# gopro/cineform-sdk

Hardware: AMD Instinct MI355X
Metric: 1080p YUY2 encode+decode fps (higher is better)
Workload: dtype int16

## Files before the change

cineform-sdk_amd/csrc/cfhd_entropy_gpu.hip:

```cpp
#include "cfhd_entropy_gpu.h"
#include "cfhd_entropy_jobs.h"
#include <hip/hip_runtime.h>
#include <string.h>
#include <stdio.h>
#include <stdlib.h>
#include <algorithm>

namespace cfhd {

int device_init();
int device_current();
namespace { int g_fail(hipError_t e, const char *what) { fprintf(stderr, "[cfhd_amd] %s: %s\n", what, hipGetErrorString(e)); return (int)e ? (int)e : -1; } }
#define HIPCHK(expr) do { hipError_t _e = (expr); if (_e != hipSuccess) return g_fail(_e, #expr); } while (0)

struct GpuEntropyEncoder::Host { EntHostJobs jobs; std::vector<EntHoleGeom> geom; dev::EntFrameJob *frames = nullptr;  };

GpuEntropyEncoder::GpuEntropyEncoder() : host_(new Host) {}
GpuEntropyEncoder::~GpuEntropyEncoder() { release(); delete host_; }

void GpuEntropyEncoder::release()
{
	(void)hipSetDevice(device_);
	void *dev[] = { d_sizes_, d_tables_, d_bands_, d_segband_, d_segs_, d_bandstate_, d_frames_, d_tmpl_, d_packed_, d_offsets_, d_tokens_, d_blocks_, d_masks_ };
	for (void *p : dev) if (p) (void)hipFree(p);
	if (h_samples_) (void)hipHostFree(h_samples_);
	if (h_sizes_) (void)hipHostFree(h_sizes_);
	if (h_offsets_) (void)hipHostFree(h_offsets_);
	d_packed_ = nullptr; d_offsets_ = h_offsets_ = nullptr;
	if (h_tmpl_) (void)hipHostFree(h_tmpl_);
	if (host_->frames) { (void)hipHostFree(host_->frames); host_->frames = nullptr; }
	for (void *&e : ev_) if (e) { (void)hipEventDestroy((hipEvent_t)e); e = nullptr; }
	for (void *&e : ev2_) if (e) { (void)hipEventDestroy((hipEvent_t)e); e = nullptr; }
	if (stream2_) { device_stream_destroy(stream2_); stream2_ = nullptr; }
	timed_ = false;
	h_samples_ = nullptr; d_sizes_ = h_sizes_ = nullptr; d_tables_ = d_bands_ = d_segband_ = d_segs_ = d_bandstate_ = d_frames_ = d_tokens_ = nullptr;
	d_tmpl_ = h_tmpl_ = nullptr; n_ = 0;
	d_blocks_ = nullptr; d_masks_ = nullptr; masks_per_frame_ = 0; use_blocks_ = false;
}

int GpuEntropyEncoder::prepare(const FramePlan &plan, int nframes, int16_t *d_coeffs, size_t stride, size_t sample_cap, void *stream)
{
	group_ = false; plan_ = plan;
	return prepare_units(nframes, d_coeffs, stride, sample_cap, stream);
}

int GpuEntropyEncoder::prepare_group(const GopPlan &plan, int ngroups, int16_t *d_coeffs, size_t stride, size_t sample_cap, void *stream)
{
	group_ = true; gplan_ = plan; plan_ = FramePlan(); plan_.interlaced = false;
	return prepare_units(ngroups, d_coeffs, stride, sample_cap, stream);
}

void GpuEntropyEncoder::build_template(const SampleHeaderInfo &hdr, SampleTemplate *t) const
{
	if (group_) build_group_template(gplan_, hdr, t); else build_sample_template(plan_, hdr, t);
}

int GpuEntropyEncoder::prepare_units(int nframes, int16_t *d_coeffs, size_t stride, size_t sample_cap, void *stream)
{
	int rc = device_init();
	if (rc) return rc;
	release();
	device_ = device_current(); (void)hipSetDevice(device_);
	const FramePlan &plan = plan_;
	n_ = nframes; cap_ = (sample_cap + 255) & ~(size_t)255; stream_ = stream; d_coeffs_ = d_coeffs; coeff_stride_ = stride;
	if (cap_ * (size_t)n_ >= ((size_t)1 << 32)) { fprintf(stderr, "[cfhd_amd] batch of %d frames exceeds the 4 GiB sample arena\n", n_); return -5; }
	{
		std::vector<dev::EntTables> h(2);
		ent_build_tables(&h[0], 1); ent_build_tables(&h[1], 2);
		HIPCHK(hipMalloc(&d_tables_, 2 * sizeof(dev::EntTables)));
		HIPCHK(hipMemcpy(d_tables_, h.data(), 2 * sizeof(dev::EntTables), hipMemcpyHostToDevice));
	}
	SampleHeaderInfo hdr0 = { 1, 2, 2, 4, !plan.interlaced, nullptr, 0, nullptr, 0 };
	tmpl_.assign(n_, SampleTemplate());
	build_template(hdr0, &tmpl_[0]);
	EntHostJobs &jobs = host_->jobs;
	host_->geom = group_ ? ent_hole_geometry(gplan_, tmpl_[0]) : ent_hole_geometry(plan, tmpl_[0]);
	const bool lists = !group_ && !plan.interlaced && plan.encoded_format == ENC_YUV422 && (plan.pixel_kind == PIX_YUY2 || plan.pixel_kind == PIX_2VUY) && plan.width % 32 == 0;
	static const int l1_seg_env = [] { const char *e = getenv("CFHD_AMD_L1_SEG"); const int v = e ? atoi(e) : 0;
	                                   return v >= dev::ENT_SEG && v <= dev::ENT_SEG_MAX && v % dev::ENT_SEG == 0 ? v : (int)dev::ENT_SEG_L1; }();
	if (!ent_build_band_jobs(host_->geom, tmpl_[0], n_, d_coeffs, stride, &jobs, lists ? l1_seg_env : (int)dev::ENT_SEG)) return -3;
	nbands_ = jobs.nbands; total_segs_ = (int)jobs.segjobs.size(); tok_per_frame_ = jobs.tok_per_frame;
	HIPCHK(hipMalloc(&d_bands_, jobs.bands.size() * sizeof(dev::EntBandJob)));
	HIPCHK(hipMemcpy(d_bands_, jobs.bands.data(), jobs.bands.size() * sizeof(dev::EntBandJob), hipMemcpyHostToDevice));
	HIPCHK(hipMalloc(&d_segband_, jobs.segjobs.size() * sizeof(dev::EntSegJob)));
	HIPCHK(hipMemcpy(d_segband_, jobs.segjobs.data(), jobs.segjobs.size() * sizeof(dev::EntSegJob), hipMemcpyHostToDevice));
	HIPCHK(hipMalloc(&d_segs_, jobs.segjobs.size() * sizeof(dev::EntSegState)));
	HIPCHK(hipMalloc(&d_tokens_, jobs.tok_per_frame * (size_t)n_ * sizeof(uint32_t)));
	HIPCHK(hipMalloc(&d_bandstate_, jobs.bands.size() * sizeof(dev::EntBandState)));
	static_assert((int)kBlockChunkCols == (int)dev::FWD_CHUNK_COLS_ENT, "one chunk geometry");
	if (lists) {
		int mask_base[kMaxChannels][kNumBands];
		masks_per_frame_ = (size_t)block_list_layout(plan, mask_base);
		HIPCHK(hipMalloc(&d_blocks_, stride * 2 * (size_t)n_));
		HIPCHK(hipMalloc((void **)&d_masks_, masks_per_frame_ * 8 * (size_t)n_ + 64));
		HIPCHK(hipMemset(d_masks_, 0, masks_per_frame_ * 8 * (size_t)n_ + 64));
	}
	HIPCHK(hipHostMalloc((void **)&h_samples_, cap_ * n_, hipHostMallocPortable));
	HIPCHK(hipMalloc((void **)&d_sizes_, sizeof(uint32_t) * 2 * n_));
	HIPCHK(hipHostMalloc((void **)&h_sizes_, sizeof(uint32_t) * 2 * n_, hipHostMallocPortable));
	memset(h_sizes_, 0, sizeof(uint32_t) * 2 * n_);
	HIPCHK(hipMalloc((void **)&d_packed_, cap_ * n_ + 256));
	HIPCHK(hipMalloc((void **)&d_offsets_, sizeof(uint32_t) * (n_ + 1)));
	HIPCHK(hipHostMalloc((void **)&h_offsets_, sizeof(uint32_t) * (n_ + 1), hipHostMallocPortable));
	memset(h_offsets_, 0, sizeof(uint32_t) * (n_ + 1));
	HIPCHK(hipMalloc((void **)&d_tmpl_, (size_t)kEntTmplStride * n_));
	HIPCHK(hipHostMalloc((void **)&h_tmpl_, (size_t)kEntTmplStride * n_, hipHostMallocPortable));
	memset(h_tmpl_, 0, (size_t)kEntTmplStride * n_);
	HIPCHK(hipMalloc(&d_frames_, n_ * sizeof(dev::EntFrameJob)));
	HIPCHK(hipHostMalloc((void **)&host_->frames, n_ * sizeof(dev::EntFrameJob), hipHostMallocPortable));
	for (int f = 0; f < n_; f++) { SampleHeaderInfo h = hdr0; h.frame_number = (uint32_t)f + 1; if ((rc = set_frame_header(f, h))) return rc; }
	for (void *&e : ev_) HIPCHK(hipEventCreate((hipEvent_t *)&e));
	for (void *&e : ev2_) HIPCHK(hipEventCreate((hipEvent_t *)&e));
	if (n_ >= 8 || !device_streams_are_lean()) HIPCHK((hipError_t)device_stream_create(&stream2_));
	return 0;
}

int GpuEntropyEncoder::set_frame_header(int f, const SampleHeaderInfo &hdr)
{
	if (f < 0 || f >= n_) return -1;
	SampleTemplate &t = tmpl_[f];
	build_template(hdr, &t);
	if (!ent_fill_frame_block(host_->geom, t, f, host_->jobs, d_coeffs_ + (size_t)f * coeff_stride_, h_tmpl_ + (size_t)kEntTmplStride * f)) return -4;
	host_->frames[f] = ent_frame_job(t, d_tmpl_ + (size_t)kEntTmplStride * f, d_packed_, (uint32_t)cap_, d_sizes_ + f, d_sizes_ + n_ + f, d_offsets_ + f);
	dirty_ = true;
	return 0;
}

int GpuEntropyEncoder::launch()
{
	(void)hipSetDevice(device_);
	hipStream_t st = (hipStream_t)stream_;
	if (dirty_) {
		HIPCHK(hipMemcpyAsync(d_tmpl_, h_tmpl_, (size_t)kEntTmplStride * n_, hipMemcpyHostToDevice, st));
		HIPCHK(hipMemcpyAsync(d_frames_, host_->frames, n_ * sizeof(dev::EntFrameJob), hipMemcpyHostToDevice, st));
		dirty_ = false;
	}
	const dev::EntTables *T = (const dev::EntTables *)d_tables_;
	const dev::EntBatchGeom geom = { total_segs_ / n_, nbands_, coeff_stride_, tok_per_frame_ };
	const int act = active_frames(), total_segs = total_segs_ / n_ * act;
	(void)hipGetLastError();
	HIPCHK(hipEventRecord((hipEvent_t)ev_[0], st));
#ifdef CFHD_AMD_PROBES
	const int count_probe = []{ const char *e = getenv("CFHD_AMD_COUNT_PROBE"); return e ? atoi(e) : 0; }();
#else
	const int count_probe = 0;
#endif
	const dev::EntBlockLists lists = { (const uint4 *)d_blocks_, d_masks_, d_coeffs_, masks_per_frame_ };
	auto count_range = [&](hipStream_t s, int lo, int n, bool level1 = false) {
		const int total = n * act;
		if (level1 && use_blocks_)
			dev::k_ent_count_blocks<<<(total + dev::ENT_WAVES - 1) / dev::ENT_WAVES, dev::ENT_THREADS, 0, s>>>((const dev::EntSegJob *)d_segband_, geom, total, (dev::EntSegState *)d_segs_, T,
			                                                                                                 d_sizes_ + n_, (uint32_t *)d_tokens_, lo, n, lists);
		else
			dev::k_ent_count<<<(total + dev::ENT_WAVES - 1) / dev::ENT_WAVES, dev::ENT_THREADS, 0, s>>>((const dev::EntSegJob *)d_segband_, geom, total, (dev::EntSegState *)d_segs_, T,
			                                                                                          d_sizes_ + n_, (uint32_t *)d_tokens_, lo, n, count_probe);
	};
	static const bool split_on = [] { const char *e = getenv("CFHD_AMD_COUNT_SPLIT"); return !(e && atoi(e) == 0); }();
	split_ = split_on && ev_level1_ && stream2_ && !host_->jobs.ranges_l1.empty() && act >= 8;
	serial_split_ = split_ && stream2_ == stream_;
	hipStream_t s1 = split_ ? (hipStream_t)stream2_ : st;
	if (s1 != st) HIPCHK(hipStreamWaitEvent(s1, (hipEvent_t)ev_level1_, 0));
	if (peak_flags_in_use()) HIPCHK(hipMemsetAsync(d_sizes_ + n_, 0, sizeof(uint32_t) * n_, s1));
	if (split_) {
// ... 643 lines not shown
```

cineform-sdk_amd/csrc/cfhd_entropy_jobs.h:

```cpp
#pragma once
#include "cfhd_core.h"
#include "cfhd_bitstream.h"
#include "cfhd_gop.h"
#include "cfhd_entropy_kernels.h"
#include "cfhd_dec_kernels.h"
#include <vector>
#include <algorithm>
#include <string.h>

namespace cfhd {

enum { kEntTmplBytes = 6144, kEntWordHolesBytes = 1536, kEntHolesBytes = dev::ENT_MAX_HOLES * (int)sizeof(dev::EntHole), kEntMaxPatches = 96,
       kEntPatchBytes = kEntMaxPatches * (int)sizeof(dev::EntPatch), kEntTmplStride = kEntTmplBytes + kEntWordHolesBytes + kEntHolesBytes + kEntPatchBytes };

inline void ent_build_tables(dev::EntTables *h, int codebook = 1)
{
	const EntropyTables *t = entropy_tables(codebook);
	memcpy(h->value_code, t->value_code, sizeof(h->value_code));
	memcpy(h->run_bits, t->run_bits, sizeof(h->run_bits));
	for (int c = 0; c < 3072; c++) { h->run_count[c] = t->run_count[c]; h->run_size[c] = t->run_size[c]; }
	h->run_total[0] = 0;
	for (int c = 1; c < 3072; c++) h->run_total[c] = (uint16_t)(t->run_size[c] + h->run_total[c - t->run_count[c]]);
	h->band_end_bits = t->band_end_bits; h->band_end_size = t->band_end_size;
	for (int c = 0; c < 3072; c++) { h->run_pack[c].x = t->run_bits[c]; h->run_pack[c].y = (uint32_t)t->run_size[c] | ((uint32_t)t->run_count[c] << 8); }
// ... 100 lines not shown
			used += total;
		}
		if (v1 && !v2) { post = mid; mid = 0; }
		const int total = pre + (v1 ? 1 : 0) + mid + (v2 ? 1 : 0) + post;
		const uint32_t o1 = v1 ? (uint32_t)pre : (uint32_t)DX_NO_VALUE, o2 = v2 ? (uint32_t)(pre + 1 + mid) : (uint32_t)DX_NO_VALUE;
		if (total > 0xfff || v1 < -128 || v1 > 127 || v2 < -128 || v2 > 127 || (v1 && pre >= (int)DX_NO_VALUE) || (v2 && pre + 1 + mid >= (int)DX_NO_VALUE)) return false;
		T->multi[win].x = (uint32_t)(used & 15) | ((uint32_t)total << 4) | (o1 << 16);
		T->multi[win].y = o2 | ((uint32_t)(uint8_t)(int8_t)v1 << 16) | ((uint32_t)(uint8_t)(int8_t)v2 << 24);
	}
	{
		auto entry_of = [&](const RawCode &c, bool *ok) {
			const uint32_t a = c.kind == 1 ? T->mag_expand[0][c.payload] : (c.kind == 0 ? (uint32_t)c.payload : 0u), b = c.kind == 1 ? T->mag_expand[1][c.payload] : a;
			const uint32_t bits = (uint32_t)c.len + (c.kind == 1 ? 1u : 0u);
			if (a >= (1u << 12) || b >= (1u << 12) || bits > 31u) *ok = false;
			return bits | ((uint32_t)type_of(c) << 5) | (a << 8) | (b << 20);
		};
		bool ok = true;
		uint32_t n11 = 0;
		int l2_of[1 << DX_KM];
		for (int p = 0; p < (1 << DX_KM); p++) l2_of[p] = -1;
		struct L3b { uint32_t key; int maxlen; uint32_t base; };
		std::vector<L3b> l3b;
		for (int i = 0; i < ncodes; i++) {
			const RawCode &c = codes[i];
			const int total = c.len + (c.kind == 1 ? 1 : 0);
			if (total <= DX_KM) continue;
			if (c.len <= DX_KM) {
				const uint32_t base = c.bits << (DX_KM - c.len);
				for (uint32_t k = 0; k < (1u << (DX_KM - c.len)); k++) { if (T->multi[base + k].x & 15u) ok = false; T->multi[base + k].y = entry_of(c, &ok); }
				continue;
			}
			const uint32_t p11 = c.bits >> (c.len - DX_KM);
			if (l2_of[p11] < 0) {
				if (n11 + (1u << DX_L11_BITS) > DX_LONG11_MAX) return false;
				l2_of[p11] = (int)n11; n11 += 1u << DX_L11_BITS;
				if (T->multi[p11].x & 15u) ok = false;
				T->multi[p11].y = (uint32_t)DX_L11_BITS | ((uint32_t)DX_T_ESCAPE << 5) | ((uint32_t)l2_of[p11] << 8);
			}
			if (c.len > DX_KM + DX_L11_BITS) {
				const uint32_t key = c.bits >> (c.len - DX_KM - DX_L11_BITS);
				auto it = std::find_if(l3b.begin(), l3b.end(), [&](const L3b &x) { return x.key == key; });
				if (it == l3b.end()) l3b.push_back(L3b{ key, c.len, 0 }); else if (c.len > it->maxlen) it->maxlen = c.len;
			}
		}
		for (L3b &x : l3b) {
			const int nb = x.maxlen - DX_KM - DX_L11_BITS;
			if (n11 + (1u << nb) > DX_LONG11_MAX) return false;
			x.base = n11; n11 += 1u << nb;
			T->long11[(uint32_t)l2_of[x.key >> DX_L11_BITS] + (x.key & ((1u << DX_L11_BITS) - 1u))] = (uint32_t)nb | ((uint32_t)DX_T_ESCAPE << 5) | (x.base << 8);
		}
		for (int i = 0; i < ncodes; i++) {
			const RawCode &c = codes[i];
			if (c.len <= DX_KM) continue;
			const uint32_t e = entry_of(c, &ok);
			if (c.len <= DX_KM + DX_L11_BITS) {
				const int spare = DX_KM + DX_L11_BITS - c.len;
				const uint32_t base = (uint32_t)l2_of[c.bits >> (c.len - DX_KM)] + ((c.bits & ((1u << (c.len - DX_KM)) - 1u)) << spare);
				for (uint32_t k = 0; k < (1u << spare); k++) T->long11[base + k] = e;
			} else {
				const uint32_t key = c.bits >> (c.len - DX_KM - DX_L11_BITS);
				const L3b &x = *std::find_if(l3b.begin(), l3b.end(), [&](const L3b &y) { return y.key == key; });
				const int nb = x.maxlen - DX_KM - DX_L11_BITS, rest = c.len - DX_KM - DX_L11_BITS, spare = nb - rest;
				const uint32_t base = x.base + ((c.bits & ((1u << rest) - 1u)) << spare);
				for (uint32_t k = 0; k < (1u << spare); k++) T->long11[base + k] = e;
			}
		}
		if (!ok) return false;
		for (uint32_t win = 0; win < (1u << DX_KM); win++) if ((T->multi[win].x & 15u) == 0 && (T->multi[win].x & 0xffffu)) return false;
	}
	return true;
}

static_assert(((size_t)dev::ENT_BLK_SPAN + 2u * (size_t)kMaxFrameDim) / 8u < ((size_t)1 << 23) && dev::ENT_BLK_SPAN / 8 <= 512, "block slot << 9 | block number fits 32 bits");

struct EntHostJobs {
	std::vector<dev::EntBandJob> bands;
	std::vector<dev::EntSegJob> segjobs;
	std::vector<int> band_of_hole;
	int nbands = 0;
	std::vector<std::pair<int, int>> ranges_l1, ranges_rest;
	size_t tok_per_frame = 0;
};

struct EntHoleGeom { size_t offset; int width, height, pitch; int table ; int mask_base ; bool level1; };
inline std::vector<EntHoleGeom> ent_hole_geometry(const FramePlan &plan, const SampleTemplate &t)
{
	int mask_base[kMaxChannels][kNumBands];
	block_list_layout(plan, mask_base);
	std::vector<EntHoleGeom> g;
	for (const SampleTemplate::Hole &hole : t.holes) {
		const BandDesc &bd = plan.ch[hole.channel].band[hole.level][hole.band];
		g.push_back(EntHoleGeom{ bd.offset, bd.width, bd.height, bd.pitch,
		                         plan.interlaced && hole.level == 0 && hole.band == 2 ? 1 : 0,
		                         hole.kind == 1 && hole.level == 0 ? mask_base[hole.channel][hole.band] : -1, hole.level == 0 });
	}
	return g;
}
inline std::vector<EntHoleGeom> ent_hole_geometry(const GopPlan &plan, const SampleTemplate &t)
{
	std::vector<EntHoleGeom> g;
	for (const SampleTemplate::Hole &hole : t.holes) {
		const GopWavelet &wv = plan.ch[hole.channel].w[hole.level];
		g.push_back(EntHoleGeom{ wv.offset[hole.band], wv.width, wv.height, wv.pitch, gop_band_is_difference_coded(plan, hole.level, hole.band) ? 1 : 0, -1, hole.level < 2 });
	}
	return g;
}

inline bool ent_build_band_jobs(const std::vector<EntHoleGeom> &geom, const SampleTemplate &t0, int nframes, int16_t *coeffs, size_t stride, EntHostJobs *out,
                                int l1_seg = dev::ENT_SEG)
{
	if ((int)t0.holes.size() > dev::ENT_MAX_HOLES || (int)t0.patches.size() > kEntMaxPatches || geom.size() != t0.holes.size()) return false;
	if (l1_seg < dev::ENT_SEG || l1_seg > dev::ENT_SEG_MAX || l1_seg % dev::ENT_SEG) return false;
	out->bands.clear(); out->segjobs.clear(); out->ranges_l1.clear(); out->ranges_rest.clear();
	out->tok_per_frame = 0;
	out->band_of_hole.assign(t0.holes.size(), -1);
	for (int f = 0; f < nframes; f++) {
		int16_t *base = coeffs + (size_t)f * stride;
		size_t tok_at = 0;
		for (size_t h = 0; h < t0.holes.size(); h++) {
			const SampleTemplate::Hole &hole = t0.holes[h];
			if (hole.kind != 1) continue;
			const EntHoleGeom &bd = geom[h];
			dev::EntBandJob j;
			j.coeffs = base + bd.offset; j.n = bd.height * bd.pitch;
			const int len = bd.level1 && bd.table == 0 && bd.mask_base >= 0 ? l1_seg : (int)dev::ENT_SEG;
			j.nseg = (j.n + len - 1) / len; j.seg_base = (int)out->segjobs.size();
			j.frame = f; j.hole = (int)h;
			j.table = bd.table;
			if (f == 0) {
				out->band_of_hole[h] = (int)out->bands.size();
				std::vector<std::pair<int, int>> &r = bd.level1 ? out->ranges_l1 : out->ranges_rest;
				if (!r.empty() && r.back().first + r.back().second == j.seg_base) r.back().second += j.nseg; else r.push_back({ j.seg_base, j.nseg });
			}
			for (int s = 0; s < j.nseg; s++) {
				const int first = s * len, slots = ((j.n - first < len ? j.n - first : len) + dev::ENT_TOK_STRIDE - 1) / dev::ENT_TOK_STRIDE * dev::ENT_TOK_STRIDE;
				out->segjobs.push_back(dev::EntSegJob{ j.coeffs, j.n, first, (int)out->bands.size(), j.table, bd.pitch, bd.mask_base, len, (int)tok_at });
				tok_at += (size_t)slots;
			}
			out->bands.push_back(j);
		}
		if (tok_at > (size_t)INT32_MAX) return false;
		out->tok_per_frame = tok_at;
	}
	out->nbands = (int)out->bands.size() / nframes;
	return true;
}
inline bool ent_build_band_jobs(const FramePlan &plan, const SampleTemplate &t0, int nframes, int16_t *coeffs, size_t stride, EntHostJobs *out, int l1_seg = dev::ENT_SEG)
{
	return ent_build_band_jobs(ent_hole_geometry(plan, t0), t0, nframes, coeffs, stride, out, l1_seg);
}

inline bool ent_fill_frame_block(const std::vector<EntHoleGeom> &geom, const SampleTemplate &t, int f, const EntHostJobs &jobs, const int16_t *coeffs_f, uint8_t *block)
{
	if (t.bytes.size() > (size_t)kEntTmplBytes || t.bytes.size() / 4 > (size_t)kEntWordHolesBytes || t.holes.size() != jobs.band_of_hole.size() ||
	    t.patches.size() > (size_t)kEntMaxPatches || geom.size() != t.holes.size()) return false;
	memcpy(block, t.bytes.data(), t.bytes.size());
	uint8_t *wh = block + kEntTmplBytes;
	size_t hole = 0;
	for (size_t w = 0; w < t.bytes.size() / 4; w++) {
		while (hole < t.holes.size() && (size_t)t.holes[hole].tmpl_offset <= w * 4) hole++;
		wh[w] = (uint8_t)hole;
	}
	dev::EntHole *eh = (dev::EntHole *)(block + kEntTmplBytes + kEntWordHolesBytes);
	for (size_t i = 0; i < t.holes.size(); i++) {
		const SampleTemplate::Hole &src = t.holes[i];
		const EntHoleGeom &bd = geom[i];
		dev::EntHole &d = eh[i];
		d.tmpl_offset = src.tmpl_offset; d.kind = src.kind; d.fixed_bytes = src.fixed_bytes;
		d.band_job = src.kind == 1 ? jobs.band_of_hole[i] + f * jobs.nbands : (src.kind == 2 && i > 0 && t.holes[i - 1].kind == 1 ? jobs.band_of_hole[i - 1] + f * jobs.nbands : -1);
		if (src.kind == 2 && d.band_job < 0) return false;
		d.lowpass = src.kind == 0 ? coeffs_f + bd.offset : nullptr;
		d.lp_width = bd.width; d.lp_height = bd.height; d.lp_pitch = bd.pitch;
	}
	dev::EntPatch *ep = (dev::EntPatch *)(block + kEntTmplBytes + kEntWordHolesBytes + kEntHolesBytes);
	for (size_t i = 0; i < t.patches.size(); i++) {
		const SampleTemplate::Patch &p = t.patches[i];
		ep[i].kind = p.kind; ep[i].at_tmpl = p.at_tmpl; ep[i].at_holes = p.at_holes; ep[i].start_tmpl = p.start_tmpl; ep[i].start_holes = p.start_holes;
		ep[i].end_tmpl = p.end_tmpl; ep[i].end_holes = p.end_holes; ep[i].tag = p.tag;
	}
	return true;
}
inline bool ent_fill_frame_block(const FramePlan &plan, const SampleTemplate &t, int f, const EntHostJobs &jobs, const int16_t *coeffs_f, uint8_t *block)
{
	return ent_fill_frame_block(ent_hole_geometry(plan, t), t, f, jobs, coeffs_f, block);
}

inline dev::EntFrameJob ent_frame_job(const SampleTemplate &t, uint8_t *block_addr, uint8_t *out, uint32_t out_cap, uint32_t *size_out, uint32_t *peak_flag, const uint32_t *dense_off = nullptr)
{
	dev::EntFrameJob fj;
	fj.out = out; fj.out_cap = out_cap; fj.dense_off = dense_off;
	fj.tmpl = block_addr; fj.tmpl_bytes = (int)t.bytes.size();
	fj.word_holes = block_addr + kEntTmplBytes;
	fj.holes = (const dev::EntHole *)(block_addr + kEntTmplBytes + kEntWordHolesBytes); fj.nholes = (int)t.holes.size();
	fj.patches = (const dev::EntPatch *)(block_addr + kEntTmplBytes + kEntWordHolesBytes + kEntHolesBytes); fj.npatches = (int)t.patches.size();
	fj.sample_bytes = size_out; fj.peak_flag = peak_flag;
	return fj;
}


inline bool dec_build_jobs(const ParsedSample &ps, const FramePlan &plan, const uint8_t *sample_addr, int16_t *coeff_base, int out_pixel_kind,
                           std::vector<dev::DecBandJob> *bands, std::vector<dev::DecLowpassJob> *lowpass, bool skip_level1 = false)
{
	for (int c = 0; c < plan.num_channels; c++) {
		const ParsedBand &lp = ps.lowpass[c];
		const BandDesc &ll = plan.ch[c].band[2][0];
		if (!lp.present || lp.width != ll.width || lp.height != ll.height) return false;
		dev::DecLowpassJob lj = { sample_addr + lp.offset, coeff_base + ll.offset, ll.width, ll.height, ll.pitch, lowpass_bias(plan.precision, ll.width, out_pixel_kind, c) };
		lowpass->push_back(lj);
		for (int lv = skip_level1 ? 1 : 0; lv < kNumLevels; lv++)
			for (int b = 1; b < 4; b++) {
				const ParsedBand &pb = ps.high[c][lv][b];
				const BandDesc &bd = plan.ch[c].band[lv][b];
				if (!pb.present || pb.width != bd.width || pb.height != bd.height || (pb.offset & 3) || (pb.codebook != 1 && pb.codebook != 0) || (bd.offset & 7) || (bd.pitch & 7)) return false;
				dev::DecBandJob bj = { sample_addr + pb.offset, pb.bytes, coeff_base + bd.offset, bd.height * bd.pitch, pb.quant };
				bands->push_back(bj);
			}
	}
	return true;
}

inline void dec_build_plan(const FramePlan &plan, int out_pixel_kind, dev::DecPlan *dp)
{
	memset(dp, 0, sizeof(*dp));
	dp->width = plan.width; dp->display_height = plan.display_height; dp->encoded_format = plan.encoded_format; dp->num_channels = plan.num_channels;
	struct Key { int area, c, lv, b; };
	std::vector<Key> keys;
	for (int c = 0; c < plan.num_channels; c++) {
		const BandDesc &ll = plan.ch[c].band[2][0];
		dp->low[c] = dev::DecPlanBand{ ll.width, ll.height, ll.pitch, (int)ll.offset };
		dp->low_bias[c] = lowpass_bias(plan.precision, ll.width, out_pixel_kind, c);
		for (int lv = 0; lv < kNumLevels; lv++)
			for (int b = 1; b < 4; b++) {
// ... 86 lines not shown
```

cineform-sdk_amd/csrc/cfhd_entropy_kernels.h:

```cpp
#pragma once
#include <stdint.h>
#include <cfhd_gfx950.h>

#ifdef CFHD_AMD_PROBES
#define CFHD_PROBE(p) (p)
#else
#define CFHD_PROBE(p) 0
#endif

namespace cfhd {
namespace dev {

#ifndef CFHD_ENT_FILL
#define CFHD_ENT_FILL 16384
#endif
#ifndef CFHD_ENT_PER_THREAD
#define CFHD_ENT_PER_THREAD 16
#endif
#ifndef CFHD_ENT_TOK_CAP
#define CFHD_ENT_TOK_CAP 256
#endif
enum { FWD_CHUNK_COLS_ENT = 496 };
enum { ENT_THREADS = 256, ENT_LANES = 64, ENT_WAVES = ENT_THREADS / ENT_LANES, ENT_PER_THREAD = CFHD_ENT_PER_THREAD, ENT_SEG = ENT_LANES * ENT_PER_THREAD,
       ENT_LDS_WORDS = 1024, ENT_TOK_CAP = CFHD_ENT_TOK_CAP, ENT_MAX_HOLES = 60 ,
       ENT_FILL = CFHD_ENT_FILL ,
       ENT_TOK_STRIDE = ENT_SEG, ENT_STR_BITS = 26, ENT_CODE_COMPLEX = 63 ,
       ENT_RUN_COMPLEX = 0xff ,
       ENT_SEG_L1 = 4096, ENT_SEG_MAX = 8192, ENT_BLK_SPAN = 4096,
       ENT_REC_RUN_SHIFT = 17 };
static_assert(ENT_SEG_MAX - 1 < (1 << (32 - ENT_REC_RUN_SHIFT)), "the longest run inside a segment fits the token record's run field");
static_assert(ENT_SEG_L1 % ENT_SEG == 0 && ENT_SEG_MAX % ENT_SEG == 0 && ENT_BLK_SPAN % ENT_SEG == 0 && ENT_BLK_SPAN / 8 <= 8 * ENT_LANES, "segments are whole token windows; a span is 8 blocks per lane");

struct EntTables {
	uint32_t value_code[2048];
	uint32_t run_bits[3072];
	uint16_t run_total[3072];
	uint16_t run_count[3072];
	uint8_t run_size[3072];
	uint32_t band_end_bits; int band_end_size;
	uint2 run_pack[3072];
};

struct EntBandJob {
	const int16_t *coeffs;
	int n;
	int seg_base, nseg;
	int frame, hole;
	int table;
};

struct EntSegJob {
	const int16_t *coeffs;
	int n;
	int first;
	int band;
	int table;
	int pitch;
	int mask_base;
	int len;
	int tok_base;
};

struct EntSegState {
	int first_nz, last_nz;
	uint32_t bits;
	int prev_nz;
	uint32_t bitoff;
	uint32_t ntok;
	uint32_t run_code, run_size;
	uint32_t run_bits;
	uint32_t lead32, lead_valid;
	uint32_t tok_blk;
	uint8_t *out;
	uint32_t info;
	uint32_t peaks;
};
static_assert(sizeof(EntSegState) == 64, "one segment state per 64 bytes");

struct EntBandState { uint32_t seg_bits, tail_run, payload_bytes, base_byte; uint8_t *out;
                      uint32_t npeaks, pad; uint8_t *peak_out;  };

struct EntHole { int tmpl_offset, kind, fixed_bytes, band_job; const int16_t *lowpass; int lp_width, lp_height, lp_pitch; };
struct EntPatch { int kind, at_tmpl, at_holes, start_tmpl, start_holes, end_tmpl, end_holes, tag; };

struct EntFrameJob {
	uint8_t *out; uint32_t out_cap;
	const uint8_t *tmpl; int tmpl_bytes;
	const uint8_t *word_holes;
	const EntHole *holes; int nholes;
	const EntPatch *patches; int npatches;
	uint32_t *sample_bytes;
	uint32_t *peak_flag;
	const uint32_t *dense_off;
};

__device__ __forceinline__ uint32_t bswap32(uint32_t v) { return (v >> 24) | ((v >> 8) & 0xff00u) | ((v << 8) & 0xff0000u) | (v << 24); }

__device__ __forceinline__ int block_excl_sum(int v, int *buf, int *total)
{
	const int lane = wave_lane(), wave = (int)(threadIdx.x >> 6);
	const int incl = (int)wave_incl_scan((uint32_t)v);
	if (lane == ENT_LANES - 1) buf[wave] = incl;
	__syncthreads();
	int base = 0, tot = 0;
#pragma unroll
	for (int w = 0; w < ENT_WAVES; w++) { const int x = buf[w]; if (w < wave) base += x; tot += x; }
	if (total) *total = tot;
	__syncthreads();
	return base + incl - v;
}
__device__ __forceinline__ int block_excl_max(int v, int *buf, int *total)
{
	const int lane = wave_lane(), wave = (int)(threadIdx.x >> 6);
// ... 63 lines not shown
}

struct EntTokCarry { int ntok, first_idx, last_idx; uint32_t bits, npeaks, lead32, lead_valid; };
__device__ __forceinline__ EntTokCarry ent_tok_carry() { EntTokCarry c; c.ntok = 0; c.first_idx = -1; c.last_idx = -1; c.bits = 0; c.npeaks = 0; c.lead32 = 0; c.lead_valid = 0; return c; }

__device__ __forceinline__ void ent_count_window(const EntSegJob &job, const EntTables *T, int nwin, int lane, const uint32_t *s_tok, uint32_t *seg_out, EntTokCarry &c, int probe)
{
	for (int t0 = 0; t0 < nwin; t0 += ENT_LANES) {
		const int t = t0 + lane;
		const bool have = t < nwin;
		const uint32_t tok = have ? s_tok[t] : 0u;
		const bool follows = have && (t > 0 || c.ntok > 0);
		const uint32_t before = follows ? (t > 0 ? s_tok[t - 1] >> 16 : (uint32_t)c.last_idx) : 0u;
		const uint32_t run = follows ? (tok >> 16) - before - 1u : 0u;
		const bool long_run = run >= 3072u;
		const uint32_t ri = long_run ? 0u : run;
		int value = (int)(int16_t)(tok & 0xffffu);
		const bool is_peak = job.table && (value > ENT_PEAK_THRESHOLD || value < -ENT_PEAK_THRESHOLD);
		if (is_peak) value = value > 0 ? ENT_PEAK_THRESHOLD + 1 : -ENT_PEAK_THRESHOLD - 1;
		c.npeaks += (uint32_t)__popcll(__ballot(is_peak));
		const uint32_t ve = value_entry(T, value);
		uint32_t rt = T->run_total[ri];
		if (__ballot(long_run)) { if (long_run) rt = run_bits_any(T, run); }
		const uint2 rp = T->run_pack[ri];
		uint32_t my_top = 0, my_len = 0;
		if (have) {
			c.bits += rt + (ve >> 27);
			const uint32_t vs = ve >> 27, vc = ve & 0x7FFFFFFu, rs = run ? rp.y & 0xffu : 0u;
			const bool simple = !long_run && (run == 0u || (rp.y >> 8) == run) && rs + vs <= (uint32_t)ENT_STR_BITS;
			const uint32_t str = simple ? (((run ? rp.x : 0u) << vs) | vc) << (32u - rs - vs) : 0u;
			const uint32_t len = simple ? rs + vs : (uint32_t)ENT_CODE_COMPLEX;
			const int v11 = value < -1023 ? -1023 : (value > 1023 ? 1023 : value);
			const uint32_t rec = simple ? str | len : (run << ENT_REC_RUN_SHIFT) | (((uint32_t)v11 & 0x7ffu) << 6) | len;
			if (CFHD_PROBE(probe) != 4) seg_out[c.ntok + t] = rec;
			my_top = str; my_len = len;
		}
		if (t0 == 0 && c.ntok == 0) {
			const int hi = nwin < ENT_LANES ? nwin : ENT_LANES;
			const unsigned long long cx = __ballot(have && my_len == (uint32_t)ENT_CODE_COMPLEX);
			const uint32_t l = (have && my_len != (uint32_t)ENT_CODE_COMPLEX) ? my_len : 0u;
			const uint32_t sc = wave_incl_scan(l), ex = sc - l;
			const int stop_lane = cx ? __builtin_ctzll(cx) : hi;
			uint32_t part = (lane < stop_lane && ex < 32u) ? my_top >> ex : 0u;
#pragma unroll
			for (int d = 1; d < ENT_LANES; d <<= 1) part |= __shfl_xor(part, d);
			c.lead32 = part;
			const uint32_t known = stop_lane > 0 ? wave_get(sc, stop_lane - 1) : 0u;
			c.lead_valid = known < 32u ? known : 32u;
		}
	}
	if (nwin) {
		if (!c.ntok) c.first_idx = (int)(s_tok[0] >> 16);
		c.last_idx = (int)(s_tok[nwin - 1] >> 16);
		c.ntok += nwin;
	}
}

__device__ __forceinline__ void ent_count_finish(int seg, const EntSegJob &job, int frame, size_t tok_base, int lane, const EntTokCarry &c, EntSegState *segs, uint32_t *peak_flags)
{
	if (c.npeaks && lane == 0) atomic_or_u32(&peak_flags[frame], 1u);
	const uint32_t bits = wave_get(wave_incl_scan(c.bits), ENT_LANES - 1);
	if (lane == 0) {
		EntSegState &s = segs[seg];
		s.first_nz = c.ntok ? job.first + c.first_idx : -1;
		s.last_nz = c.ntok ? job.first + c.last_idx : -1;
		s.bits = bits;
		s.ntok = (uint32_t)c.ntok;
		s.lead32 = c.lead32; s.lead_valid = c.lead_valid;
		s.tok_blk = (uint32_t)(tok_base / ENT_TOK_STRIDE);
		s.out = nullptr;
		s.info = (job.first != 0 ? 1u : 0u) | (job.first + job.len < job.n ? 2u : 0u) | ((uint32_t)job.table << 8);
		s.peaks = c.npeaks;
	}
}

__device__ __forceinline__ void ent_count_segment(int seg, const EntSegJob &job, int frame, size_t tok_base, uint32_t *w, int lane, uint32_t *s_tok, EntSegState *segs, const EntTables *tables,
                                                  uint32_t *peak_flags, uint32_t *tokens, int probe)
{
	if (CFHD_PROBE(probe) == 1) { uint32_t o = 0; for (int j = 0; j < ENT_SEG / 128; j++) o |= w[j]; const unsigned long long q = __ballot(o == 0x12345u); if (lane == 0) { EntSegState &z = segs[seg]; z.first_nz = -1; z.last_nz = -1; z.bits = q == 0x123456789ull; z.ntok = 0; z.lead32 = 0; z.lead_valid = 0; } return; }
	const EntTables *T = tables + job.table;
	EntTokCarry c = ent_tok_carry();
	const int span = job.n - job.first < job.len ? job.n - job.first : job.len;
	for (int off = 0; off < span; off += ENT_SEG) {
		if (off) ent_load_segment(job, lane, w, off);
		int nwin = 0;
#pragma unroll
		for (int j = 0; j < ENT_SEG / 128; j++) {
			const uint32_t vl = w[j] & 0xffffu, vh = w[j] >> 16;
			const unsigned long long ml = __ballot(vl != 0u), mh = __ballot(vh != 0u);
			const int pl = nwin + (int)wave_mbcnt(ml) + (int)wave_mbcnt(mh);
			const uint32_t idx = (uint32_t)(off + j * 128 + 2 * lane) << 16;
			if (vl) s_tok[pl] = idx | vl;
			if (vh) s_tok[pl + (vl != 0u)] = (idx + 0x10000u) | vh;
			nwin += __popcll(ml) + __popcll(mh);
		}
		CFHD_WAVE_SYNC();
		if (CFHD_PROBE(probe) == 2) { const unsigned long long q = __ballot(s_tok[lane] == 0x12345u); if (lane == 0) { EntSegState &z = segs[seg]; z.first_nz = -1; z.last_nz = -1; z.bits = q == 0x123456789ull && nwin == 0x12345; z.ntok = 0; z.lead32 = 0; z.lead_valid = 0; } return; }
		ent_count_window(job, T, nwin, lane, s_tok, tokens + tok_base, c, probe);
		CFHD_WAVE_SYNC();
	}
	ent_count_finish(seg, job, frame, tok_base, lane, c, segs, peak_flags);
}

enum { ENT_COUNT_SEGS = 1 };
__global__ void __launch_bounds__(ENT_THREADS) k_ent_count(const EntSegJob *seg_jobs, EntBatchGeom geom, int total_segs, EntSegState *segs, const EntTables *tables,
                                                            uint32_t *peak_flags, uint32_t *tokens, int range_lo, int range_n,
                                                            int probe = 0 )
{
	__shared__ uint32_t s_tok_all[ENT_WAVES][ENT_SEG];
	const int lane = wave_lane();
	const int wave = wave_uniform((int)(threadIdx.x >> 6));
	const int idx0 = wave_uniform(((int)blockIdx.x * ENT_WAVES + wave) * ENT_COUNT_SEGS);
	if (idx0 >= total_segs) return;
	const int seg0 = (idx0 / range_n) * geom.segs_per_frame + range_lo + idx0 % range_n;
	static_assert(ENT_COUNT_SEGS == 1, "the range mapping takes one segment per wave");
	EntSegJob job[ENT_COUNT_SEGS]; int frame[ENT_COUNT_SEGS]; size_t tok_base[ENT_COUNT_SEGS];
	uint32_t w[ENT_COUNT_SEGS][ENT_SEG / 128];
#pragma unroll
	for (int k = 0; k < ENT_COUNT_SEGS; k++)
		if (idx0 + k < total_segs) { job[k] = ent_seg_job(seg_jobs, geom, seg0 + k, &frame[k], &tok_base[k]); ent_load_segment(job[k], lane, w[k]); }
#pragma unroll
	for (int k = 0; k < ENT_COUNT_SEGS; k++)
		if (idx0 + k < total_segs) {
			ent_count_segment(seg0 + k, job[k], frame[k], tok_base[k], w[k], lane, s_tok_all[wave], segs, tables, peak_flags, tokens, probe);
			CFHD_WAVE_SYNC();
		}
}

struct EntBlockLists { const uint4 *blocks; const unsigned long long *masks; const int16_t *coeff0; size_t masks_per_frame; };
__global__ void __launch_bounds__(ENT_THREADS) k_ent_count_blocks(const EntSegJob *seg_jobs, EntBatchGeom geom, int total_segs, EntSegState *segs, const EntTables *tables,
                                                                   uint32_t *peak_flags, uint32_t *tokens, int range_lo, int range_n, EntBlockLists lists)
{
	__shared__ uint32_t s_tok_all[ENT_WAVES][ENT_SEG];
	enum { SPAN_BLOCKS = ENT_BLK_SPAN / 8, HMAX = SPAN_BLOCKS / ENT_LANES };
	const int lane = wave_lane();
	const int wave = wave_uniform((int)(threadIdx.x >> 6));
	const int idx0 = wave_uniform((int)blockIdx.x * ENT_WAVES + wave);
	if (idx0 >= total_segs) return;
	const int seg = (idx0 / range_n) * geom.segs_per_frame + range_lo + idx0 % range_n;
	int frame; size_t tok_base;
	const EntSegJob job = ent_seg_job(seg_jobs, geom, seg, &frame, &tok_base);
	const EntTables *T = tables + job.table;
	uint32_t *s_tok = s_tok_all[wave], *seg_out = tokens + tok_base;
	const int pitch = job.pitch, cpr = (pitch + FWD_CHUNK_COLS_ENT - 1) / FWD_CHUNK_COLS_ENT;
	const int seg_end = job.first + job.len, end = seg_end < job.n ? seg_end : job.n;
	const uint4 *band_blocks = lists.blocks + (size_t)(job.coeffs - lists.coeff0) / 8;
	const unsigned long long *masks = wave_uniform_ptr(lists.masks + (size_t)frame * lists.masks_per_frame + job.mask_base);
	EntTokCarry c = ent_tok_carry();
	for (int s0 = job.first; s0 < end; s0 += ENT_BLK_SPAN) {
		const int nq = (seg_end - s0 < ENT_BLK_SPAN ? seg_end - s0 : ENT_BLK_SPAN) / 8;
		const int row0 = s0 / pitch, col0 = s0 - row0 * pitch;
		const uint4 *blocks = wave_uniform_ptr(band_blocks + (size_t)row0 * (size_t)(pitch >> 3));
		uint32_t entry[HMAX]; bool listed[HMAX];
		int row = 0, col = col0 + 8 * lane;
		while (col >= pitch) { col -= pitch; row++; }
#pragma unroll
		for (int h = 0; h < HMAX; h++) {
			listed[h] = false; entry[h] = 0u;
			if (ENT_LANES * h >= nq) continue;
			if (h) { col += 8 * ENT_LANES; while (col >= pitch) { col -= pitch; row++; } }
			const int q = lane + ENT_LANES * h, pos = s0 + 8 * q;
			static_assert(FWD_CHUNK_COLS_ENT == 62 * 8, "the division below is by 62 blocks");
			const uint32_t c8 = (uint32_t)col >> 3, k = mul_u24(c8, 1058u) >> 16, i = c8 - mul_u24(k, 62u);
			unsigned long long m = 0ull;
			if (pos < end) m = masks[mul_u24((uint32_t)(row0 + row), (uint32_t)cpr) + k];
			listed[h] = ((m >> i) & 1ull) != 0ull;
			entry[h] = ((mul_u24((uint32_t)row, (uint32_t)pitch >> 3) + mul_u24(k, 62u) + (uint32_t)__popcll(m & ((1ull << i) - 1ull))) << 9) | (uint32_t)q;
		}
		int nlisted = 0;
#pragma unroll
		for (int h = 0; h < HMAX; h++) {
			if (ENT_LANES * h >= nq) break;
			const unsigned long long b = __ballot(listed[h]);
			if (listed[h]) s_tok[nlisted + (int)wave_mbcnt(b)] = entry[h];
			nlisted += __popcll(b);
		}
		CFHD_WAVE_SYNC();
		uint32_t mine[HMAX];
#pragma unroll
		for (int h = 0; h < HMAX; h++) mine[h] = lane + ENT_LANES * h < nlisted ? s_tok[lane + ENT_LANES * h] : 0u;
		CFHD_WAVE_SYNC();
		int nwin = 0;
// ... 259 lines not shown
			put_code_plain(words, pos, T->band_end_bits, T->band_end_size);
		}
	}
}

__device__ __forceinline__ void ent_put_string(uint32_t *s_words, uint32_t *out, bool use_lds, uint32_t first_word, uint64_t pos, uint64_t str)
{
	const uint32_t sh = (uint32_t)pos & 31u, w = (uint32_t)(pos >> 5);
	const uint64_t top = str >> sh;
	const uint32_t a = (uint32_t)(top >> 32), b = (uint32_t)top, c = (uint32_t)(((uint64_t)(uint32_t)str << 32) >> sh);
	if (use_lds) {
		atomic_or_u32(&s_words[w - first_word], a);
		if (b) atomic_or_u32(&s_words[w - first_word + 1], b);
		if (c) atomic_or_u32(&s_words[w - first_word + 2], c);
	} else {
		atomic_or_u32(&out[w], bswap32(a));
		if (b) atomic_or_u32(&out[w + 1], bswap32(b));
		if (c) atomic_or_u32(&out[w + 2], bswap32(c));
	}
}

__device__ __forceinline__ void ent_put_string32(uint32_t *s_words, uint32_t *out, bool use_lds, uint32_t first_word, uint64_t pos, uint32_t str)
{
	const uint32_t sh = (uint32_t)pos & 31u, w = (uint32_t)(pos >> 5);
	const uint32_t a = str >> sh, b = sh ? str << (32u - sh) : 0u;
	if (use_lds) {
		atomic_or_u32(&s_words[w - first_word], a);
		if (b) atomic_or_u32(&s_words[w - first_word + 1], b);
	} else {
		atomic_or_u32(&out[w], bswap32(a));
		if (b) atomic_or_u32(&out[w + 1], bswap32(b));
	}
}

__device__ __forceinline__ void ent_put_long_run(const EntTables *T, uint32_t *s_words, uint32_t *out, bool use_lds, uint32_t first_word, uint64_t pos, uint32_t run, int owner)
{
	const int lane = wave_lane();
	const uint32_t cmax = T->run_count[3071], smax = T->run_size[3071], codemax = T->run_bits[3071];
	const uint32_t nrep = run >= 3072u ? (run - 3072u) / cmax + 1u : 0u;
	for (uint32_t i = (uint32_t)lane; i < nrep; i += ENT_LANES) ent_put_string(s_words, out, use_lds, first_word, pos + (uint64_t)i * smax, (uint64_t)codemax << (64u - smax));
	if (lane == owner) {
		uint32_t left = run - nrep * cmax;
		pos += (uint64_t)nrep * smax;
		while (left > 0u) {
			const uint2 rc = T->run_pack[left < 3072u ? left : 3071u];
			const uint32_t size = rc.y & 0xffu;
			ent_put_string(s_words, out, use_lds, first_word, pos, (uint64_t)rc.x << (64u - size));
			pos += size; left -= rc.y >> 8;
		}
	}
}

__device__ __forceinline__ bool ent_ordinary(const EntSegState &st)
{
	return st.bits >= 32u && (uint32_t)((st.bitoff + st.bits - 1u) >> 5) - (uint32_t)(st.bitoff >> 5) + 1u <= (uint32_t)ENT_LDS_WORDS;
}
__device__ __forceinline__ bool ent_neighbours_merge(const EntSegState &a, const EntSegState &b)
{
	const uint32_t o = b.bitoff & 31u;
	return o != 0u && ent_ordinary(a) && ent_ordinary(b) && b.lead_valid >= 32u - o;
}

__device__ __forceinline__ void ent_emit_segment(const EntSegState &st, const EntSegState &pv, const EntSegState &nx, const uint32_t first_rec, const uint32_t *seg_str, int lane,
                                                 uint32_t *s_words, const EntTables *tables, int probe)
{
	if (st.bits == 0) return;
	const EntTables *T = tables + (st.info >> 8);
	const bool has_prev = (st.info & 1u) != 0u, has_next = (st.info & 2u) != 0u;
	const bool prev_writes_first = has_prev && ent_neighbours_merge(pv, st);
	const bool merge_next = has_next && ent_neighbours_merge(st, nx);
	uint32_t *out = (uint32_t *)st.out;
	if (!out) return;
	if (CFHD_PROBE(probe) == 2) { if (first_rec == 0x12345u && lane == 0) out[0] = 1; return; }
	const int ntok = (int)st.ntok;
	const uint64_t seg_pos = st.bitoff;
	const uint32_t first_word = (uint32_t)(seg_pos >> 5), last_word = (uint32_t)((seg_pos + st.bits - 1) >> 5);
	const uint32_t nwords = last_word - first_word + 1;
	const bool use_lds = nwords <= ENT_LDS_WORDS;
	if (use_lds) for (int i = lane; i < (int)nwords + 2; i += ENT_LANES) s_words[i] = 0;
	CFHD_WAVE_SYNC();
	if (st.run_size == (uint32_t)ENT_RUN_COMPLEX) ent_put_long_run(T, s_words, out, use_lds, first_word, seg_pos, (uint32_t)(st.first_nz - st.prev_nz - 1), 0);
	else if (st.run_size && lane == 0) ent_put_string(s_words, out, use_lds, first_word, seg_pos, (uint64_t)st.run_code << (64u - st.run_size));
	uint64_t round_pos = seg_pos + st.run_bits;
	for (int t = lane, t0 = 0; t0 < ntok; t0 += ENT_LANES, t += ENT_LANES) {
		const bool have = t < ntok;
		uint32_t rec = t0 == 0 ? first_rec : seg_str[have ? t : 0];
		if (!have) rec = 0u;
		uint32_t len = rec & 63u;
		const bool complex = len == (uint32_t)ENT_CODE_COMPLEX;
		uint32_t run = 0, ve = 0;
		if (__ballot(complex)) {
			if (complex) {
				run = rec >> ENT_REC_RUN_SHIFT;
				ve = value_entry(T, (int)(rec << (32 - ENT_REC_RUN_SHIFT)) >> 21);
				len = run_bits_any(T, run) + (ve >> 27);
			}
		}
		const uint32_t sc = wave_incl_scan(len);
		uint64_t pos = round_pos + (sc - len);
		round_pos += wave_get(sc, ENT_LANES - 1);
		if (have && !complex) ent_put_string32(s_words, out, use_lds, first_word, pos, rec & ~63u);
		if (complex) {
			uint32_t left = run;
			while (left > 0u) {
				const uint2 rc = T->run_pack[left < 3072u ? left : 3071u];
				const uint32_t size = rc.y & 0xffu;
				ent_put_string(s_words, out, use_lds, first_word, pos, (uint64_t)rc.x << (64u - size));
				pos += size; left -= rc.y >> 8;
			}
			ent_put_string(s_words, out, use_lds, first_word, pos, (uint64_t)(ve & 0x7FFFFFFu) << (64u - (ve >> 27)));
		}
	}
	CFHD_WAVE_SYNC();
	if (CFHD_PROBE(probe) == 3) { if (s_words[lane] == 0x12345u) out[0] = 1; return; }
	if (use_lds) {
		const bool first_shared = (seg_pos & 31u) != 0u, last_shared = ((seg_pos + st.bits) & 31u) != 0u;
		for (int i = lane; i < (int)nwords; i += ENT_LANES) {
			uint32_t w = s_words[i];
			const bool is_first = i == 0, is_last = i == (int)nwords - 1;
			if (is_first && prev_writes_first) continue;
			if (is_last && merge_next) w |= nx.lead32 >> ((seg_pos + st.bits) & 31u);
			w = bswap32(w);
			if (((is_first && first_shared) || (is_last && last_shared && !merge_next)) && CFHD_PROBE(probe) != 4) { if (w) atomic_or_u32(&out[first_word + i], w); }
			else if (CFHD_PROBE(probe) != 5) out[first_word + i] = w;
		}
	}
}

enum { ENT_EMIT_SEGS = 1 };
__global__ void __launch_bounds__(ENT_THREADS) k_ent_emit(int total_segs, const EntSegState *segs, const EntTables *tables, const uint32_t *tokens,
                                                           int probe = 0 )
{
	__shared__ uint32_t s_words_all[ENT_WAVES][ENT_LDS_WORDS + 3];
	if (CFHD_PROBE(probe) == 1) return;
	const int lane = wave_lane();
	const int wave = wave_uniform((int)(threadIdx.x >> 6));
	const int seg0 = wave_uniform(((int)blockIdx.x * ENT_WAVES + wave) * ENT_EMIT_SEGS);
	if (seg0 >= total_segs) return;
	uint32_t first_rec[ENT_EMIT_SEGS];
	EntSegState st[ENT_EMIT_SEGS + 2];
#pragma unroll
	for (int k = 0; k < ENT_EMIT_SEGS + 2; k++) {
		int sg = seg0 - 1 + k;
		sg = sg < 0 ? 0 : (sg < total_segs ? sg : total_segs - 1);
		st[k] = segs[sg];
	}
#pragma unroll
	for (int k = 0; k < ENT_EMIT_SEGS; k++)
		first_rec[k] = tokens[(size_t)st[k + 1].tok_blk * ENT_TOK_STRIDE + lane];
#pragma unroll
	for (int k = 0; k < ENT_EMIT_SEGS; k++)
		if (seg0 + k < total_segs) {
			ent_emit_segment(st[k + 1], st[k], st[k + 2], first_rec[k], tokens + (size_t)st[k + 1].tok_blk * ENT_TOK_STRIDE, lane, s_words_all[wave], tables, probe);
			CFHD_WAVE_SYNC();
		}
}


struct EntPeakHoles { int n; int hole[7]; };
__global__ void __launch_bounds__(ENT_THREADS) k_ent_peaks(const EntFrameJob *frames, EntPeakHoles which, const EntBandJob *bands, const EntSegJob *seg_jobs, EntBatchGeom geom,
                                                            const EntSegState *segs, const EntBandState *band_state)
{
	const EntHole &hole = frames[blockIdx.z].holes[which.hole[blockIdx.y]];
	const int bj = hole.band_job, quant = hole.fixed_bytes;
	const EntBandState bs = band_state[bj];
	if (!bs.npeaks || !bs.peak_out || bs.npeaks > (uint32_t)ENT_PEAK_TABLE_MAX) return;
	const EntBandJob band = bands[bj];
	int16_t *table = (int16_t *)bs.peak_out;
	const int lane = wave_lane();
	const int wave = wave_uniform((int)(threadIdx.x >> 6));
// ... 520 lines not shown
```

Baseline: 66680.

## Use longer entropy segments for dense bands and prefetch next window loads

```diff
diff --git a/cineform-sdk_amd/csrc/cfhd_entropy_gpu.hip b/cineform-sdk_amd/csrc/cfhd_entropy_gpu.hip
--- a/cineform-sdk_amd/csrc/cfhd_entropy_gpu.hip
+++ b/cineform-sdk_amd/csrc/cfhd_entropy_gpu.hip
@@ -78,7 +78,11 @@
 	const bool lists = !group_ && !plan.interlaced && plan.encoded_format == ENC_YUV422 && (plan.pixel_kind == PIX_YUY2 || plan.pixel_kind == PIX_2VUY) && plan.width % 32 == 0;
 	static const int l1_seg_env = [] { const char *e = getenv("CFHD_AMD_L1_SEG"); const int v = e ? atoi(e) : 0;
 	                                   return v >= dev::ENT_SEG && v <= dev::ENT_SEG_MAX && v % dev::ENT_SEG == 0 ? v : (int)dev::ENT_SEG_L1; }();
-	if (!ent_build_band_jobs(host_->geom, tmpl_[0], n_, d_coeffs, stride, &jobs, lists ? l1_seg_env : (int)dev::ENT_SEG)) return -3;
+	enum { kWaveSlots = 256 * 4 * 8 };
+	const bool fills_chip = (size_t)n_ * stride / dev::ENT_SEG >= (size_t)kWaveSlots;
+	auto seg_env = [&](const char *name, int dflt) { const char *e = getenv(name); const int v = e ? atoi(e) : 0; return ent_seg_len_ok(v) ? v : (fills_chip ? dflt : (int)dev::ENT_SEG); };
+	const EntSegRule rule = { seg_env("CFHD_AMD_SEG_L1_DENSE", dev::ENT_SEG_L1_DENSE), seg_env("CFHD_AMD_SEG_L2", dev::ENT_SEG_L2), seg_env("CFHD_AMD_SEG_L3", dev::ENT_SEG_L3), lists };
+	if (!ent_build_band_jobs(host_->geom, tmpl_[0], n_, d_coeffs, stride, &jobs, lists ? l1_seg_env : (int)dev::ENT_SEG, &rule)) return -3;
 	nbands_ = jobs.nbands; total_segs_ = (int)jobs.segjobs.size(); tok_per_frame_ = jobs.tok_per_frame;
 	HIPCHK(hipMalloc(&d_bands_, jobs.bands.size() * sizeof(dev::EntBandJob)));
 	HIPCHK(hipMemcpy(d_bands_, jobs.bands.data(), jobs.bands.size() * sizeof(dev::EntBandJob), hipMemcpyHostToDevice));
diff --git a/cineform-sdk_amd/csrc/cfhd_entropy_jobs.h b/cineform-sdk_amd/csrc/cfhd_entropy_jobs.h
--- a/cineform-sdk_amd/csrc/cfhd_entropy_jobs.h
+++ b/cineform-sdk_amd/csrc/cfhd_entropy_jobs.h
@@ -206,7 +206,8 @@
 	size_t tok_per_frame = 0;
 };
 
-struct EntHoleGeom { size_t offset; int width, height, pitch; int table ; int mask_base ; bool level1; };
+struct EntHoleGeom { size_t offset; int width, height, pitch; int table ; int mask_base ; bool level1;
+                     int level ; };
 inline std::vector<EntHoleGeom> ent_hole_geometry(const FramePlan &plan, const SampleTemplate &t)
 {
 	int mask_base[kMaxChannels][kNumBands];
@@ -216,7 +217,7 @@
 		const BandDesc &bd = plan.ch[hole.channel].band[hole.level][hole.band];
 		g.push_back(EntHoleGeom{ bd.offset, bd.width, bd.height, bd.pitch,
 		                         plan.interlaced && hole.level == 0 && hole.band == 2 ? 1 : 0,
-		                         hole.kind == 1 && hole.level == 0 ? mask_base[hole.channel][hole.band] : -1, hole.level == 0 });
+		                         hole.kind == 1 && hole.level == 0 ? mask_base[hole.channel][hole.band] : -1, hole.level == 0, hole.level + 1 });
 	}
 	return g;
 }
@@ -225,16 +226,20 @@
 	std::vector<EntHoleGeom> g;
 	for (const SampleTemplate::Hole &hole : t.holes) {
 		const GopWavelet &wv = plan.ch[hole.channel].w[hole.level];
-		g.push_back(EntHoleGeom{ wv.offset[hole.band], wv.width, wv.height, wv.pitch, gop_band_is_difference_coded(plan, hole.level, hole.band) ? 1 : 0, -1, hole.level < 2 });
+		g.push_back(EntHoleGeom{ wv.offset[hole.band], wv.width, wv.height, wv.pitch, gop_band_is_difference_coded(plan, hole.level, hole.band) ? 1 : 0, -1, hole.level < 2,
+		                         hole.level < 2 ? 1 : (hole.level < 5 ? 2 : 3) });
 	}
 	return g;
 }
 
+struct EntSegRule { int l1_dense, l2, l3; bool lists; };
+inline bool ent_seg_len_ok(int v) { return v >= dev::ENT_SEG && v <= dev::ENT_SEG_MAX && v % dev::ENT_SEG == 0; }
+
 inline bool ent_build_band_jobs(const std::vector<EntHoleGeom> &geom, const SampleTemplate &t0, int nframes, int16_t *coeffs, size_t stride, EntHostJobs *out,
-                                int l1_seg = dev::ENT_SEG)
+                                int l1_seg = dev::ENT_SEG, const EntSegRule *rule = nullptr)
 {
 	if ((int)t0.holes.size() > dev::ENT_MAX_HOLES || (int)t0.patches.size() > kEntMaxPatches || geom.size() != t0.holes.size()) return false;
-	if (l1_seg < dev::ENT_SEG || l1_seg > dev::ENT_SEG_MAX || l1_seg % dev::ENT_SEG) return false;
+	if (!ent_seg_len_ok(l1_seg) || (rule && !(ent_seg_len_ok(rule->l1_dense) && ent_seg_len_ok(rule->l2) && ent_seg_len_ok(rule->l3)))) return false;
 	out->bands.clear(); out->segjobs.clear(); out->ranges_l1.clear(); out->ranges_rest.clear();
 	out->tok_per_frame = 0;
 	out->band_of_hole.assign(t0.holes.size(), -1);
@@ -247,7 +252,8 @@
 			const EntHoleGeom &bd = geom[h];
 			dev::EntBandJob j;
 			j.coeffs = base + bd.offset; j.n = bd.height * bd.pitch;
-			const int len = bd.level1 && bd.table == 0 && bd.mask_base >= 0 ? l1_seg : (int)dev::ENT_SEG;
+			int len = bd.level1 && bd.table == 0 && bd.mask_base >= 0 ? l1_seg : (int)dev::ENT_SEG;
+			if (rule && bd.table == 0 && !(bd.level1 && bd.mask_base >= 0 && rule->lists)) len = bd.level1 ? rule->l1_dense : (bd.level <= 2 ? rule->l2 : rule->l3);
 			j.nseg = (j.n + len - 1) / len; j.seg_base = (int)out->segjobs.size();
 			j.frame = f; j.hole = (int)h;
 			j.table = bd.table;
@@ -269,9 +275,10 @@
 	out->nbands = (int)out->bands.size() / nframes;
 	return true;
 }
-inline bool ent_build_band_jobs(const FramePlan &plan, const SampleTemplate &t0, int nframes, int16_t *coeffs, size_t stride, EntHostJobs *out, int l1_seg = dev::ENT_SEG)
-{
-	return ent_build_band_jobs(ent_hole_geometry(plan, t0), t0, nframes, coeffs, stride, out, l1_seg);
+inline bool ent_build_band_jobs(const FramePlan &plan, const SampleTemplate &t0, int nframes, int16_t *coeffs, size_t stride, EntHostJobs *out, int l1_seg = dev::ENT_SEG,
+                                const EntSegRule *rule = nullptr)
+{
+	return ent_build_band_jobs(ent_hole_geometry(plan, t0), t0, nframes, coeffs, stride, out, l1_seg, rule);
 }
 
 inline bool ent_fill_frame_block(const std::vector<EntHoleGeom> &geom, const SampleTemplate &t, int f, const EntHostJobs &jobs, const int16_t *coeffs_f, uint8_t *block)
diff --git a/cineform-sdk_amd/csrc/cfhd_entropy_kernels.h b/cineform-sdk_amd/csrc/cfhd_entropy_kernels.h
--- a/cineform-sdk_amd/csrc/cfhd_entropy_kernels.h
+++ b/cineform-sdk_amd/csrc/cfhd_entropy_kernels.h
@@ -27,8 +27,10 @@
        ENT_TOK_STRIDE = ENT_SEG, ENT_STR_BITS = 26, ENT_CODE_COMPLEX = 63 ,
        ENT_RUN_COMPLEX = 0xff ,
        ENT_SEG_L1 = 4096, ENT_SEG_MAX = 8192, ENT_BLK_SPAN = 4096,
+       ENT_SEG_L1_DENSE = 4096, ENT_SEG_L2 = 2048, ENT_SEG_L3 = 1024,
        ENT_REC_RUN_SHIFT = 17 };
 static_assert(ENT_SEG_MAX - 1 < (1 << (32 - ENT_REC_RUN_SHIFT)), "the longest run inside a segment fits the token record's run field");
+static_assert(ENT_SEG_L1_DENSE % ENT_SEG == 0 && ENT_SEG_L2 % ENT_SEG == 0 && ENT_SEG_L3 % ENT_SEG == 0 && ENT_SEG_L1_DENSE <= ENT_SEG_MAX && ENT_SEG_L2 <= ENT_SEG_MAX && ENT_SEG_L3 <= ENT_SEG_MAX, "dense segments are whole token windows too");
 static_assert(ENT_SEG_L1 % ENT_SEG == 0 && ENT_SEG_MAX % ENT_SEG == 0 && ENT_BLK_SPAN % ENT_SEG == 0 && ENT_BLK_SPAN / 8 <= 8 * ENT_LANES, "segments are whole token windows; a span is 8 blocks per lane");
 
 struct EntTables {
@@ -258,7 +260,9 @@
 	EntTokCarry c = ent_tok_carry();
 	const int span = job.n - job.first < job.len ? job.n - job.first : job.len;
 	for (int off = 0; off < span; off += ENT_SEG) {
-		if (off) ent_load_segment(job, lane, w, off);
+		const bool more = off + ENT_SEG < span;
+		uint32_t wn[ENT_SEG / 128];
+		if (more) ent_load_segment(job, lane, wn, off + ENT_SEG);
 		int nwin = 0;
 #pragma unroll
 		for (int j = 0; j < ENT_SEG / 128; j++) {
@@ -274,6 +278,10 @@
 		if (CFHD_PROBE(probe) == 2) { const unsigned long long q = __ballot(s_tok[lane] == 0x12345u); if (lane == 0) { EntSegState &z = segs[seg]; z.first_nz = -1; z.last_nz = -1; z.bits = q == 0x123456789ull && nwin == 0x12345; z.ntok = 0; z.lead32 = 0; z.lead_valid = 0; } return; }
 		ent_count_window(job, T, nwin, lane, s_tok, tokens + tok_base, c, probe);
 		CFHD_WAVE_SYNC();
+		if (more) {
+#pragma unroll
+			for (int j = 0; j < ENT_SEG / 128; j++) w[j] = wn[j];
+		}
 	}
 	ent_count_finish(seg, job, frame, tok_base, lane, c, segs, peak_flags);
 }
@@ -699,10 +707,11 @@
 	if (st.run_size == (uint32_t)ENT_RUN_COMPLEX) ent_put_long_run(T, s_words, out, use_lds, first_word, seg_pos, (uint32_t)(st.first_nz - st.prev_nz - 1), 0);
 	else if (st.run_size && lane == 0) ent_put_string(s_words, out, use_lds, first_word, seg_pos, (uint64_t)st.run_code << (64u - st.run_size));
 	uint64_t round_pos = seg_pos + st.run_bits;
+	uint32_t next_rec = first_rec;
 	for (int t = lane, t0 = 0; t0 < ntok; t0 += ENT_LANES, t += ENT_LANES) {
 		const bool have = t < ntok;
-		uint32_t rec = t0 == 0 ? first_rec : seg_str[have ? t : 0];
-		if (!have) rec = 0u;
+		uint32_t rec = have ? next_rec : 0u;
+		if (t0 + ENT_LANES < ntok) next_rec = seg_str[t + ENT_LANES < ntok ? t + ENT_LANES : 0];
 		uint32_t len = rec & 63u;
 		const bool complex = len == (uint32_t)ENT_CODE_COMPLEX;
 		uint32_t run = 0, ve = 0;
```

Result: faster. 67930 (median of 6 runs) (+1.9%).
